# zjwzcx/A-2D-LiDAR-based-SLAM-System-for-Wheeled-Mobile-Robots

Hardware: AMD Instinct MI355X
Metric: scans/sec (360-beam ICP + 0.05 m grid update) (higher is better)
Workload: dtype f64; 1 GPU; configs[1]: 1000-scan replay (every 5th message of a 10 Hz stream, seed 1), 360 beams, ICP(max_iter=30, tol=0.001) + 400x400@0.05m grid, f64 point buffers; 32 independent replays of the 1000-scan trajectory per step (one slam_replay_dev call: ranges [32, 1000, 360], a map per trajectory); point_buffers=f64, pipeline=0, lanes=2, grid_mode=1, grid_group=16, parallelism=1 trajectory per GPU (32 independent replays of it per step)

## Files before the change

### a-2d-lidar-based-slam-system-for-wheeled-mobile-robots_amd/csrc/grid_kernels.hip

```cpp
#include <hip/hip_runtime.h>

#include <algorithm>
#include <mutex>
#include <utility>
#include <vector>
#include <climits>
#include <type_traits>

#include "slam_internal.h"
#include "slam_stamps.h"
#include "grid_walk.h"

namespace slam {

__device__ __forceinline__ unsigned cast_ray(uint32_t *__restrict__ pass, uint32_t *__restrict__ hit, int xw, int yw,
                                             int pcx, int pcy, int pox, int poy, bool &first_pending)
{
    Ray r;
    first_pending = false;
    if (!ray_setup(pcx, pcy, pox, poy, r)) return 0u;
    unsigned nvis = 0;
    double error = 0.0;
    int y = r.y0;
    for (int k = 0; k <= r.dx; ++k) {
        int x = r.x0 + k;
        int lx = r.steep ? y : x, ly = r.steep ? x : y;
        bool last = r.flag ? (k == 0) : (k == r.dx);
        bool first = r.flag ? (k == r.dx) : (k == 0);
        if ((unsigned)lx < (unsigned)xw && (unsigned)ly < (unsigned)yw) {
            ++nvis;
            if (first && lx == pcx && ly == pcy) {
                first_pending = true;
            } else {
                size_t c = (size_t)lx * yw + ly;
                atomicAdd(last ? &hit[c] : &pass[c], 1u);
            }
        }
        if (walk_step(error, r.derr)) y += r.ystep;
    }
    return nvis;
}

__device__ __forceinline__ unsigned wave_sum_u32(unsigned v)
{
#pragma unroll
    for (int off = 32; off > 0; off >>= 1) v += __shfl_xor(v, off, kWave);
    return v;
}

__device__ __forceinline__ int wave_or_i32(int v)
{
#pragma unroll
    for (int off = 32; off > 0; off >>= 1) v |= __shfl_xor(v, off, kWave);
    return v;
}

__device__ __forceinline__ void finish_wave(const GridDev &g, uint32_t *pass, int pcx, int pcy, bool first_pending,
                                            unsigned nvis, int bad)
{
    unsigned long long m = __ballot(first_pending);
    unsigned tot = wave_sum_u32(nvis);
    const int anybad = wave_or_i32(bad);
    if ((threadIdx.x & 63) == 0) {
        if (m) atomicAdd(&pass[(size_t)pcx * g.yw + pcy], (unsigned)__popcll(m));
        if (tot) atomicAdd(visit_slot(g.visits), (unsigned long long)tot);
        if (anybad) atomicOr(g.status, anybad);
    }
}

__device__ __forceinline__ void owner_fence() { asm volatile("s_waitcnt vmcnt(0)" ::: "memory"); }
constexpr int kWinCells = 36864;
constexpr int kWinMaxGroup = 64;
constexpr int kSortBins = 128;
constexpr int kMaxSortRays = 8192;
constexpr int kRaysPerLane = 4;

struct ScanConst {
    double px, py, c, s;
    int pcx, pcy, cbad, pad;
};

struct ReplaySource {
    const float *ranges;
    const double *cos_t, *sin_t, *poses;
    int n_scan, n;
    long traj_stride;
    int grid_per_traj;
    const double *centres;
    const double *heading_cs = nullptr;
    __device__ int scans_per_traj() const { return n_scan - 1; }
    __device__ int own_grid(int l) const { return grid_per_traj ? l : 0; }
    bool maps_are_private() const { return grid_per_traj != 0; }
    ReplaySource trajectories_from(int l0) const
    {
        ReplaySource r = *this;
        const size_t k = (size_t)l0 * (n_scan - 1);
        r.ranges += (size_t)l0 * traj_stride; r.poses += 3 * k;
        if (centres) r.centres += 2 * k;
        if (heading_cs) r.heading_cs += 2 * k;
        return r;
    }
    ReplaySource scans_from(int k0, int cnt) const
    {
        ReplaySource r = *this;
        r.ranges += (size_t)k0 * n; r.poses += 3 * (size_t)k0;
        if (centres) r.centres += 2 * (size_t)k0;
        if (heading_cs) r.heading_cs += 2 * (size_t)k0;
        r.n_scan = cnt + 1;
        return r;
    }
    __device__ void scan_const(int l, int k, const GridDev &g, ScanConst &sc) const
    {
        const double *pose = poses + 3 * ((size_t)l * (n_scan - 1) + k);
        sc.px = pose[0]; sc.py = pose[1];
        if (heading_cs) {
            const double *cs = heading_cs + 2 * ((size_t)l * (n_scan - 1) + k);
            sc.c = cs[0]; sc.s = cs[1];
        } else {
            sc.c = cos(pose[2]); sc.s = sin(pose[2]);
        }
        sc.cbad = 0;
        double ox = sc.px, oy = sc.py;
        if (centres) {
            const double *ctr = centres + 2 * ((size_t)l * (n_scan - 1) + k);
            ox = ctr[0]; oy = ctr[1];
        }
        sc.pcx = to_cell(ox, g.scale, g.off_x, sc.cbad);
        sc.pcy = to_cell(oy, g.scale, g.off_y, sc.cbad);
    }
    struct Beam { float r; double ct, st; };
    __device__ Beam fetch(int l, int k, int i) const
    {
        return Beam{ranges[(size_t)l * traj_stride + (size_t)(k + 1) * n + i], cos_t[i], sin_t[i]};
    }
    __device__ bool ray(const Beam &b, const ScanConst &sc, const GridDev &g, int &pox, int &poy, int &bad) const
    {
        double rr = (double)b.r;
        if (rr == INFINITY) rr = 30.0;
        double lx = b.ct * rr, ly = b.st * rr;
        double x = sc.c * lx + (-sc.s) * ly + sc.px * 1.0;
        double y = sc.s * lx + sc.c * ly + sc.py * 1.0;
        if (fabs(x) == INFINITY) return false;
        pox = to_cell(x, g.scale, g.off_x, bad);
        poy = to_cell(y, g.scale, g.off_y, bad);
        bad |= sc.cbad;
        return !bad;
    }
    __device__ bool ray(int l, int k, int i, const ScanConst &sc, const GridDev &g, int &pox, int &poy, int &bad) const
    {
        return ray(fetch(l, k, i), sc, g, pox, poy, bad);
    }
};

struct ExplicitSource {
    const double *ox, *oy, *cx, *cy;
    int B, n;
    __device__ int scans_per_traj() const { return B; }
    __device__ int own_grid(int) const { return 0; }
    bool maps_are_private() const { return false; }
// ... 54 lines not shown
        if (i < n && i <= stop && src.ray(l, k, i, sc, g, pox, poy, bad))
            nvis = cast_ray(pass, hit, g.xw, g.yw, sc.pcx, sc.pcy, pox, poy, first_pending);
        finish_wave(g, pass, sc.pcx, sc.pcy, first_pending, nvis, bad);
    }
}

typedef __attribute__((address_space(3))) unsigned lds_u32_t;
__device__ __forceinline__ unsigned lds_addr(const void *p)
{
    return (unsigned)(uintptr_t)(__attribute__((address_space(3))) const void *)p;
}
__device__ __forceinline__ void lds_add_u32(unsigned addr, unsigned v)
{
    (void)__hip_atomic_fetch_add((lds_u32_t *)(uintptr_t)addr, v, __ATOMIC_RELAXED, __HIP_MEMORY_SCOPE_WORKGROUP);
}

__device__ __forceinline__ int wave_min_i32(int v)
{
#pragma unroll
    for (int off = 32; off > 0; off >>= 1) v = min(v, __shfl_xor(v, off, kWave));
    return v;
}
__device__ __forceinline__ int wave_max_i32(int v)
{
#pragma unroll
    for (int off = 32; off > 0; off >>= 1) v = max(v, __shfl_xor(v, off, kWave));
    return v;
}

__device__ __forceinline__ void lds_walk(unsigned a, int da_k, int da_y, int rem, double derr, double &error, bool lead_in)
{
    auto advance = [&]() {
        const bool stepy = walk_step(error, derr);
        a += (unsigned)(da_k + (stepy ? da_y : 0));
    };
    auto step = [&]() {
        lds_add_u32(a & ~3u, 1u << ((a << 3) & 31u));
        advance();
    };
    if (lead_in) advance();
    for (;;) {
        const bool full = rem >= 4;
        if (!__any(full)) break;
        if (full) { step(); step(); step(); step(); rem -= 4; }
    }
#pragma unroll
    for (int u = 0; u < 3; ++u)
        if (rem > u) step();
}

__device__ __forceinline__ bool next_rays(int *next_ray, int nrays, const unsigned short *order, int &r)
{
    const int lane = threadIdx.x & 63;
    int base = 0;
    if (lane == 0) base = atomicAdd(next_ray, kWave);
    base = __builtin_amdgcn_readfirstlane(base);
    if (base >= nrays) return false;
    r = base + lane >= nrays ? -1 : order ? (int)order[base + lane] : base + lane;
    return true;
}

template <bool COVERS, class Src>
__device__ __forceinline__ unsigned cast_rays(const GridDev &g, const Src &src, const ScanConst *sc, int l, int s0, int n,
                                              int nrays, int *next_ray, const unsigned short *order, unsigned *win, int wx0,
                                              int wy0, int W, int H, int Hp2, uint32_t *__restrict__ pass,
                                              uint32_t *__restrict__ hit, const int *first_bad)
{
    unsigned nvis = 0;
    for (int r; next_rays(next_ray, nrays, order, r);) {
        if (r < 0) continue;
        int s = r / n, i = r - s * n, pox, poy, b2 = 0;
        Ray ry;
        if (i >= first_bad[s]) continue;
        if (!src.ray(l, s0 + s, i, sc[s], g, pox, poy, b2)) continue;
        if (!ray_setup(sc[s].pcx, sc[s].pcy, pox, poy, ry)) continue;
        CellWalk w(ry);
        int hx = -1, hy = -1;
        const int Hs = 2 * Hp2;
        const bool safe = (unsigned)(sc[s].pcx - wx0) < (unsigned)W && (unsigned)(sc[s].pcy - wy0) < (unsigned)H &&
                    (unsigned)(pox - wx0) < (unsigned)W && (unsigned)(poy - wy0) < (unsigned)H;
        if (!__any(!safe)) {
            const unsigned a2 = lds_addr(win) + 2u * (unsigned)((w.lx - wx0) * Hs + (w.ly - wy0));
            nvis += (unsigned)ry.dx + 1u;
            lds_walk(a2, 2 * w.stride_k(Hs), 2 * w.stride_y(Hs), ry.dx, w.derr, w.error, ry.flag);
            atomicAdd(&hit[(size_t)pox * g.yw + poy], 1u);
            continue;
        }
        for (int k = 0; k <= ry.dx; ++k, w.next()) {
            const int lx = w.lx, ly = w.ly;
            bool last = k == w.klast;
            unsigned wx = (unsigned)(lx - wx0), wy = (unsigned)(ly - wy0);
            bool inwin = wx < (unsigned)W && wy < (unsigned)H;
            bool inmap = COVERS ? inwin : ((unsigned)lx < (unsigned)g.xw && (unsigned)ly < (unsigned)g.yw);
            nvis += inmap ? 1u : 0u;
            hx = last ? lx : hx; hy = last ? ly : hy;
            if (inwin && !last) atomicAdd(&win[wx * Hp2 + (wy >> 1)], 1u << ((wy & 1u) * 16u));
            if (!COVERS) { if (inmap && !inwin && !last) atomicAdd(&pass[(size_t)lx * g.yw + ly], 1u); }
        }
        if ((unsigned)hx < (unsigned)g.xw && (unsigned)hy < (unsigned)g.yw) atomicAdd(&hit[(size_t)hx * g.yw + hy], 1u);
    }
    return nvis;
}

template <class Src>
__device__ __forceinline__ unsigned cast_rays_strip(const GridDev &g, const Src &src, const ScanConst &sc, int l, int s0,
                                                    int nrays, int *next_ray, const unsigned short *order, unsigned *win,
                                                    int wx0, int wy0, int W, int H, int Hp2, uint32_t *__restrict__ hit,
                                                    int first_bad)
{
    unsigned nvis = 0;
    for (int i; next_rays(next_ray, nrays, order, i);) {
        if (i < 0) continue;
        int pox, poy, b2 = 0;
        Ray ry;
        if (i >= first_bad) continue;
        if (!src.ray(l, s0, i, sc, g, pox, poy, b2)) continue;
        if (max(sc.pcx, pox) < wx0 || min(sc.pcx, pox) >= wx0 + W) continue;
        if (!ray_setup(sc.pcx, sc.pcy, pox, poy, ry)) continue;
        CellWalk w(ry);
        for (int k = 0; k <= ry.dx; ++k, w.next()) {
            const unsigned wx = (unsigned)(w.lx - wx0), wy = (unsigned)(w.ly - wy0);
            if (wx < (unsigned)W && wy < (unsigned)H) {
                ++nvis;
                unsigned *cell = &win[wx * Hp2 + (wy >> 1)];
                const unsigned sh = (wy & 1u) * 16u;
                if (k != w.klast) atomicAdd(cell, 1u << sh);
                else { atomicOr(cell, 0x8000u << sh); atomicAdd(&hit[(size_t)w.lx * g.yw + w.ly], 1u); }
            }
        }
    }
    return nvis;
}

struct WinCtl {
    int bbox[4];
    int qbox[4][4];
    int next_ray;
    int strips, strip_w;
    int phases, parity;
    alignas(8) unsigned long long visits;
    int first_bad[kWinMaxGroup];
    int phw[4][8];
    int phq[4];
    int seg[5];
};
constexpr int kWinBoxInts = 160;
static_assert(sizeof(WinCtl) <= kWinBoxInts * 4 && alignof(WinCtl) <= 16, "the control block outgrew its LDS region");
__host__ __device__ inline size_t win_sc_bytes(int group) { return ((size_t)group * sizeof(ScanConst) + 15) & ~(size_t)15; }
__host__ __device__ inline int win_sort_cap(long rays) { return rays <= kMaxSortRays ? (int)((rays + 7) & ~7L) : 0; }
__host__ __device__ inline size_t win_lds_bytes(int group, int sort_cap, int win_cells)
{
    return win_sc_bytes(group) + kWinBoxInts * 4 + 4 * kSortBins * 4 + (size_t)sort_cap * 2 + (size_t)win_cells * 2 + kLdsGuard;
}
inline int win_cells_for(int group, int sort_cap)
{
    const long half = 80 * 1024 - 512;
    long other = (long)win_lds_bytes(group, sort_cap, 0);
    long cells = ((half - other) / 2) & ~15L;
    return cells > kWinCells ? (int)cells : kWinCells;
}

struct WinLds {
    ScanConst *sc; WinCtl *ctl; int *hist; unsigned short *order; unsigned *win; char *guard;
    __device__ __forceinline__ WinLds(char *smem, int group_size, int sort_cap, int win_cells)
        : sc(reinterpret_cast<ScanConst *>(smem)),
          ctl(reinterpret_cast<WinCtl *>(smem + win_sc_bytes(group_size))),
          hist(reinterpret_cast<int *>(ctl) + kWinBoxInts),
          order(reinterpret_cast<unsigned short *>(hist + 4 * kSortBins)),
          win(reinterpret_cast<unsigned *>(order + sort_cap)),
          guard(reinterpret_cast<char *>(win) + (size_t)win_cells * 2) {}
};

template <class Src, class Park>
__device__ __forceinline__ void win_pass1(const GridDev &g, const Src &src, const ScanConst *sc, int l, int s0, int cnt, int n,
                                          bool sorted, int *bbox, int *first_bad, Park &&park)
{
    const int tid = threadIdx.x;
    int bx0 = INT_MAX, by0 = INT_MAX, bx1 = INT_MIN, by1 = INT_MIN;
    for (int r = tid; r < cnt * n; r += blockDim.x) {
        int s = r / n, i = r - s * n, pox, poy, len = 0, b2 = 0, quad = 0;
        const bool valid = src.ray(l, s0 + s, i, sc[s], g, pox, poy, b2);
        if (valid) {
            quad = (pox >= sc[s].pcx ? 1 : 0) | (poy >= sc[s].pcy ? 2 : 0);
            const int rx0 = min(pox, sc[s].pcx), rx1 = max(pox, sc[s].pcx), ry0 = min(poy, sc[s].pcy), ry1 = max(poy, sc[s].pcy);
            bx0 = min(bx0, rx0); bx1 = max(bx1, rx1);
            by0 = min(by0, ry0); by1 = max(by1, ry1);
            len = max(abs(pox - sc[s].pcx), abs(poy - sc[s].pcy));
        }
        if (b2) atomicMin(&first_bad[s], i);
        if (sorted) park(r, i, valid && len > 0, quad, kSortBins - 1 - min(len >> 2, kSortBins - 1));
    }
    bx0 = wave_min_i32(bx0); by0 = wave_min_i32(by0); bx1 = wave_max_i32(bx1); by1 = wave_max_i32(by1);
    if ((tid & 63) == 0 && bx0 <= bx1) {
        atomicMin(&bbox[0], bx0); atomicMin(&bbox[1], by0); atomicMax(&bbox[2], bx1); atomicMax(&bbox[3], by1);
    }
    __syncthreads();
    if (tid < cnt && first_bad[tid] != INT_MAX) {
        int pox, poy, b2 = 0;
        (void)src.ray(l, s0 + tid, first_bad[tid], sc[tid], g, pox, poy, b2);
        atomicOr(g.status, b2);
    }
}

template <int kBinsPerLane>
__device__ __forceinline__ void counting_sort(int *hist, const unsigned short *bins, unsigned short *order, int nrays, int *seg)
{
    constexpr int kLanesPerSeg = kSortBins / kBinsPerLane;
    const int lane = threadIdx.x & 63;
    if (threadIdx.x < kWave) {
        int h[kBinsPerLane], tot = 0;
#pragma unroll
        for (int u = 0; u < kBinsPerLane; ++u) { h[u] = hist[kBinsPerLane * lane + u]; tot += h[u]; }
        int inc = tot;
#pragma unroll
        for (int off = 1; off < kWave; off <<= 1) { int v = __shfl_up(inc, off, kWave); if (lane >= off) inc += v; }
        int run = inc - tot;
        if (seg && lane % kLanesPerSeg == 0) seg[lane / kLanesPerSeg] = run;
        if (seg && lane == kWave - 1) seg[kWave / kLanesPerSeg] = inc;
#pragma unroll
        for (int u = 0; u < kBinsPerLane; ++u) { hist[kBinsPerLane * lane + u] = run; run += h[u]; }
    }
    __syncthreads();
    for (int r = threadIdx.x; r < nrays; r += blockDim.x)
        if (bins[r] != 0xffffu) order[atomicAdd(&hist[bins[r]], 1)] = (unsigned short)r;
    __syncthreads();
}

__device__ __forceinline__ bool clamp_box(const GridDev &g, int *o, int ymask)
{
    o[0] = max(o[0], 0); o[1] = max(o[1], 0); o[2] = min(o[2], g.xw - 1); o[3] = min(o[3], g.yw - 1);
    o[1] &= ~ymask;
    return o[0] <= o[2] && o[1] <= o[3];
}
__device__ __forceinline__ bool box_fits(const int *o, int win_cells)
{
    return (long)(o[2] - o[0] + 1) * ((o[3] - o[1] + 2) & ~1) <= win_cells;
}

__device__ __forceinline__ void fit_window(const GridDev &g, bool any, const int *o, int ymask, const ScanConst &first, int win_cells, int *w)
{
    int x0 = any ? o[0] : 0, y0 = any ? o[1] : 0, W = any ? o[2] - o[0] + 1 : 0, H = any ? o[3] - o[1] + 1 : 0, cov = 1;
    if (any && !box_fits(o, win_cells)) {
        const int Hd = min(H, 192), Wd = min(W, win_cells / ((Hd + 1) & ~1));
        x0 = min(max(first.pcx - Wd / 2, o[0]), o[2] - Wd + 1);
        y0 = min(max(first.pcy - Hd / 2, o[1]), o[3] - Hd + 1) & ~ymask;
        W = Wd; H = Hd; cov = 0;
    }
    if ((long)W * ((H + 1) >> 1) > win_cells / 2) { atomicOr(g.status, kStatusGuard); W = 0; H = 0; cov = 0; }
    w[0] = x0; w[1] = y0; w[2] = W; w[3] = H; w[4] = cov;
}

__device__ __forceinline__ void flush_window(const unsigned *win, uint32_t *pass, int yw, int wx0, int wy0, int W, int Hp2, bool pair64)
{
    const int lane = threadIdx.x & 63, wave = threadIdx.x >> 6, nwaves = blockDim.x >> 6;
    const int rot = W > 0 ? (int)((blockIdx.x * 37u + blockIdx.y * 11u) % (unsigned)W) : 0;
    for (int rr = wave; rr < W; rr += nwaves) {
        const int row = rr + rot < W ? rr + rot : rr + rot - W;
        size_t gbase = (size_t)(wx0 + row) * yw + wy0;
        if (pair64 && (wy0 & 1) == 0) {
            for (int d = lane; d < Hp2; d += kWave) {
                unsigned v = win[row * Hp2 + d];
                if (v) atomicAdd(reinterpret_cast<unsigned long long *>(&pass[gbase + 2 * d]),
                                 (unsigned long long)(v & 0xffffu) | ((unsigned long long)(v >> 16) << 32));
            }
            continue;
        }
        for (int d = lane; d < Hp2; d += kWave) {
            unsigned v = win[row * Hp2 + d];
            unsigned p0 = v & 0xffffu, p1 = v >> 16;
            if (p0) atomicAdd(&pass[gbase + 2 * d], p0);
            if (p1) atomicAdd(&pass[gbase + 2 * d + 1], p1);
        }
    }
}

__device__ __forceinline__ void sweep_strip(const unsigned *win, uint32_t *pass, int8_t *pm, int yw, int sx0, int wy0, int SW, int H,
                                            int qrow, unsigned qinv, uint32_t pthr)
{
    const int tid = threadIdx.x, lane = tid & 63, Hp2 = H >> 1, total = SW * qrow;
    constexpr int kBatch = 4;
    for (int q0 = tid; q0 < total; q0 += kBatch * blockDim.x) {
        uint4 p[kBatch];
        uint32_t om[kBatch], d0[kBatch], d1[kBatch];
        size_t at[kBatch];
        bool live[kBatch];
#pragma unroll
        for (int u = 0; u < kBatch; ++u) {
            const int q = q0 + u * (int)blockDim.x;
            d0[u] = d1[u] = 0u;
            if (q < total) {
                const int r = (int)__umulhi((unsigned)q, qinv), c = q - r * qrow;
                const uint2 d = *reinterpret_cast<const uint2 *>(win + (r * Hp2 + 2 * c));
                d0[u] = d.x; d1[u] = d.y;
                at[u] = (size_t)(sx0 + r) * yw + (wy0 + 4 * c);
            }
            const unsigned long long m = __ballot((d0[u] | d1[u]) != 0u);
            live[u] = ((m >> (lane & 60)) & 0xFull) != 0ull;
            if (live[u]) {
                p[u] = *reinterpret_cast<const uint4 *>(pass + at[u]);
                om[u] = *reinterpret_cast<const uint32_t *>(pm + at[u]);
            }
        }
#pragma unroll
        for (int u = 0; u < kBatch; ++u) {
            if (!live[u]) continue;
            const uint32_t d0v = d0[u], d1v = d1[u];
            p[u].x += d0v & 0x7fffu; p[u].y += (d0v >> 16) & 0x7fffu; p[u].z += d1v & 0x7fffu; p[u].w += (d1v >> 16) & 0x7fffu;
            *reinterpret_cast<uint4 *>(pass + at[u]) = p[u];
            if (!(d0v | d1v)) continue;
            const uint32_t o = om[u];
            const uint32_t tb = ((d0v & 0xffffu) ? 1u : 0u) | ((d0v >> 16) ? 0x100u : 0u) | ((d1v & 0xffffu) ? 0x10000u : 0u) | ((d1v >> 16) ? 0x1000000u : 0u);
            const uint32_t fb = ((d0v >> 15) & 1u) | (((d0v >> 31) & 1u) << 8) | (((d1v >> 15) & 1u) << 16) | ((d1v >> 31) << 24);
            const uint32_t was = (o >> 6) & 0x01010101u, fresh = (o >> 4) & 0x01010101u;
            const uint32_t pmax = max(max(p[u].x, p[u].y), max(p[u].z, p[u].w));
            if (((tb & ~was) & (fresh | fb)) != 0u || pmax >= pthr) {
                uint32_t occ = was | fb;
                occ |= (p[u].x >= pthr ? 1u : 0u) | (p[u].y >= pthr ? 0x100u : 0u) | (p[u].z >= pthr ? 0x10000u : 0u) | (p[u].w >= pthr ? 0x1000000u : 0u);
                const uint32_t tm = tb * 255u;
                const uint32_t out = (o & ~tm) | ((occ * 100u) & tm);
                if (out != o) *reinterpret_cast<uint32_t *>(pm + at[u]) = out;
            }
        }
    }
}

__device__ __forceinline__ void finish_workgroup(const GridDev &g, unsigned long long *wg_visits, unsigned nvis, int tid)
{
    const unsigned tot = wave_sum_u32(nvis);
    if ((tid & 63) == 0 && tot) atomicAdd(wg_visits, (unsigned long long)tot);
    __syncthreads();
    if (tid == 0 && *wg_visits) atomicAdd(visit_slot(g.visits), *wg_visits);
}

template <class Src>
__global__ void __launch_bounds__(1024) k_grid_update_win(GridDev g, Src src, int group_size, const int32_t *__restrict__ got,
                                                          int sort_cap, int win_cells, int split)
{
    extern __shared__ __attribute__((aligned(16))) char smem[];
    const WinLds lds(smem, group_size, sort_cap, win_cells);
    ScanConst *sc = lds.sc; WinCtl *ctl = lds.ctl; int *hist = lds.hist; unsigned *win = lds.win;
    lds_guard_fill(lds.guard);
    STAMP_DECL;

    const int tid = threadIdx.x;
    const int l = blockIdx.y;
    const int my_half = split ? (int)(blockIdx.x & 1u) : -1;
    const int s0 = (int)(split ? blockIdx.x >> 1 : blockIdx.x) * group_size;
    const int cnt = min(group_size, src.scans_per_traj() - s0);
    const int gi = got ? got[l] : src.own_grid(l);
    uint32_t *pass = g.pass + (size_t)gi * g.xw * g.yw, *hit = g.hit + (size_t)gi * g.xw * g.yw;
    const int n = src.n, nrays = cnt * n;

    const bool pair64 = (g.yw & 1) == 0 && (((size_t)gi * g.xw * g.yw) & 1) == 0;
    const int ymask = pair64 ? 1 : 0;
    if (tid < cnt) { src.scan_const(l, s0 + tid, g, sc[tid]); ctl->first_bad[tid] = INT_MAX; }
    if (tid == 0) {
        ctl->bbox[0] = ctl->bbox[1] = INT_MAX; ctl->bbox[2] = ctl->bbox[3] = INT_MIN; ctl->next_ray = 0; ctl->visits = 0ull;
        for (int q = 0; q < 4; ++q) { ctl->qbox[q][0] = ctl->qbox[q][1] = INT_MAX; ctl->qbox[q][2] = ctl->qbox[q][3] = INT_MIN; }
        ctl->phases = 1; ctl->parity = 0;
    }
    const bool sorted = nrays <= sort_cap;
    unsigned short *bins = reinterpret_cast<unsigned short *>(win);
    for (int k = tid; k < 4 * kSortBins; k += blockDim.x) hist[k] = 0;
    __syncthreads();
    STAMP(0);

    win_pass1(g, src, sc, l, s0, cnt, n, sorted, ctl->bbox, ctl->first_bad, [&](int r, int i, bool casts, int quad, int lbin) {
        bins[r] = casts ? (unsigned short)(lbin | (quad << 7) | ((i & 1) << 9)) : (unsigned short)0xffffu;
    });
    if (tid == 0) {
        const int *bb = ctl->bbox;
        if (bb[0] <= bb[2]) {
            int ox0 = INT_MAX, oy0 = INT_MAX, ox1 = INT_MIN, oy1 = INT_MIN;
            for (int k = 0; k < cnt; ++k) { ox0 = min(ox0, sc[k].pcx); ox1 = max(ox1, sc[k].pcx); oy0 = min(oy0, sc[k].pcy); oy1 = max(oy1, sc[k].pcy); }
            for (int q = 0; q < 4; ++q) {
                ctl->qbox[q][0] = (q & 1) ? max(ox0, bb[0]) : bb[0]; ctl->qbox[q][2] = (q & 1) ? bb[2] : min(ox1, bb[2]);
                ctl->qbox[q][1] = (q & 2) ? max(oy0, bb[1]) : bb[1]; ctl->qbox[q][3] = (q & 2) ? bb[3] : min(oy1, bb[3]);
            }
        }
        auto box_of = [&](unsigned mask, int *o) -> bool {
            o[0] = o[1] = INT_MAX; o[2] = o[3] = INT_MIN;
            for (int q = 0; q < 4; ++q) {
                const int *b = ctl->qbox[q];
                if ((mask >> q & 1u) && b[0] <= b[2]) { o[0] = min(o[0], b[0]); o[1] = min(o[1], b[1]); o[2] = max(o[2], b[2]); o[3] = max(o[3], b[3]); }
            }
            return clamp_box(g, o, ymask);
        };
        auto fits = [&](unsigned mask) -> bool { int o[4]; return !box_of(mask, o) || box_fits(o, win_cells); };
        unsigned part[4] = {0u, 0u, 0u, 0u};
        int nph = 1, parity = 0;
        if (split) {
            const unsigned mine = my_half ? 0xAu : 0x5u;
            if (fits(0xFu)) { part[0] = 0xFu; parity = 1; }
            else if (fits(mine)) part[0] = mine;
            else { part[0] = mine & 0x3u; part[1] = mine & 0xCu; nph = 2; }
        } else {
            if (!sorted || fits(0xFu)) part[0] = 0xFu;
            else if (fits(0x5u) && fits(0xAu)) { part[0] = 0x5u; part[1] = 0xAu; nph = 2; }
            else { part[0] = 1u; part[1] = 2u; part[2] = 4u; part[3] = 8u; nph = 4; }
        }
        for (int q = 0; q < 4; ++q) ctl->phq[q] = -1;
        for (int ph = 0; ph < nph; ++ph) {
            for (int q = 0; q < 4; ++q)
                if (part[ph] >> q & 1u) ctl->phq[q] = ph;
            int o[4];
            const bool any = box_of(part[ph], o);
            fit_window(g, any, o, ymask, sc[0], win_cells, ctl->phw[ph]);
        }
        ctl->phases = nph; ctl->parity = parity;
        if (!sorted) { ctl->seg[0] = 0; ctl->seg[1] = nrays; }
    }
    __syncthreads();
    STAMP(1);
    const int phases = ctl->phases;
    if (sorted) {
        const bool parity = ctl->parity != 0;
        for (int r = tid; r < nrays; r += blockDim.x) {
            const unsigned b = bins[r];
            if (b == 0xffffu) continue;
            const int ph = ctl->phq[(b >> 7) & 3u];
            const bool mine = ph >= 0 && (!parity || (int)((b >> 9) & 1u) == my_half);
            const unsigned fin = (unsigned)ph * kSortBins + (b & 127u);
            bins[r] = mine ? (unsigned short)fin : (unsigned short)0xffffu;
            if (mine) atomicAdd(&hist[fin], 1);
        }
        __syncthreads();
        counting_sort<8>(hist, bins, lds.order, nrays, ctl->seg);
    }
    unsigned nvis = 0;
    int W = ctl->phw[0][2], H = ctl->phw[0][3];
    bool covers = ctl->phw[0][4] != 0;
    for (int ph = 0; ph < phases; ++ph) {
        const int seg0 = ctl->seg[ph], seg1 = ctl->seg[ph + 1];
        if (seg0 == seg1) continue;
        const int *o = ctl->phw[ph];
        const int wx0 = o[0], wy0 = o[1];
        W = o[2]; H = o[3]; covers = o[4] != 0;
        const int Hp2 = (H + 1) >> 1;
        __syncthreads();
        if (tid == 0) ctl->next_ray = 0;
        for (int w = tid; w < W * Hp2; w += blockDim.x) win[w] = 0u;
        __syncthreads();
        STAMP(2);
        const unsigned short *ord = sorted ? lds.order + seg0 : nullptr;
        if (covers) nvis += cast_rays<true>(g, src, sc, l, s0, n, seg1 - seg0, &ctl->next_ray, ord, win, wx0, wy0, W, H, Hp2, pass, hit, ctl->first_bad);
        else        nvis += cast_rays<false>(g, src, sc, l, s0, n, seg1 - seg0, &ctl->next_ray, ord, win, wx0, wy0, W, H, Hp2, pass, hit, ctl->first_bad);
        __syncthreads();
        STAMP(3);
        flush_window(win, pass, g.yw, wx0, wy0, W, Hp2, pair64);
    }
    finish_workgroup(g, &ctl->visits, nvis, tid);
    STAMP(4);
    STAMP_VAL((ctl->parity << 8) | (covers ? 1 : 0) | (phases << 4) | ((unsigned)(W * ((H + 1) & ~1)) << 12));
    STAMP_END(5);
    lds_guard_check(lds.guard, g.status);
}

template <class Src>
__global__ void __launch_bounds__(1024) k_grid_update_own(GridDev g, Src src, int group_size, int sort_cap, int win_cells)
{
    extern __shared__ __attribute__((aligned(16))) char smem[];
    const WinLds lds(smem, group_size, sort_cap, win_cells);
    ScanConst *sc = lds.sc; WinCtl *ctl = lds.ctl; int *hist = lds.hist; unsigned *win = lds.win;
    lds_guard_fill(lds.guard);
    STAMP_DECL;

    const int tid = threadIdx.x, lane = tid & 63, wave = tid >> 6, nwaves = blockDim.x >> 6;
    const int l = blockIdx.y;
    const int s0 = (int)blockIdx.x * group_size;
    const int cnt = min(group_size, src.scans_per_traj() - s0);
    const int gi = src.own_grid(l);
    uint32_t *pass = g.pass + (size_t)gi * g.xw * g.yw, *hit = g.hit + (size_t)gi * g.xw * g.yw;
    int8_t *pm = g.pmap_live + (size_t)gi * g.xw * g.yw;
    const int n = src.n, nrays = cnt * n;

    const bool fused = (g.yw & 3) == 0 && (((size_t)gi * g.xw * g.yw) & 3) == 0;
    const bool pair64 = (g.yw & 1) == 0 && (((size_t)gi * g.xw * g.yw) & 1) == 0;
    const int ymask = fused ? 3 : pair64 ? 1 : 0;
    if (tid < cnt) { src.scan_const(l, s0 + tid, g, sc[tid]); ctl->first_bad[tid] = INT_MAX; }
    if (tid == 0) {
        ctl->bbox[0] = ctl->bbox[1] = INT_MAX; ctl->bbox[2] = ctl->bbox[3] = INT_MIN; ctl->next_ray = 0; ctl->visits = 0ull;
        ctl->strips = 0; ctl->strip_w = 0;
    }
    const bool sorted = nrays <= sort_cap;
    unsigned short *bins = reinterpret_cast<unsigned short *>(win);
    for (int k = tid; k < kSortBins; k += blockDim.x) hist[k] = 0;
    __syncthreads();
    STAMP(0);

    win_pass1(g, src, sc, l, s0, cnt, n, sorted, ctl->bbox, ctl->first_bad, [&](int r, int, bool, int, int lbin) {
        bins[r] = (unsigned short)lbin;
        atomicAdd(&hist[lbin], 1);
    });
    if (tid == 0) {
        int o[4] = {ctl->bbox[0], ctl->bbox[1], ctl->bbox[2], ctl->bbox[3]};
        int *w = ctl->phw[0];
        const bool any = clamp_box(g, o, 0);
        if (any && fused && cnt == 1 && nrays < 32768 && g.hit_levels == 1 && (g.yw & 15) == 0) {
            const int ya = o[1] & ~15, Ha = ((o[3] | 15) + 1) - ya, Wb = o[2] - o[0] + 1;
            int S = (int)(((long)Wb * Ha + win_cells - 1) / win_cells), Ws = (Wb + S - 1) / S;
            while ((long)Ws * Ha > win_cells && S < Wb) { ++S; Ws = (Wb + S - 1) / S; }
            if ((long)Ws * Ha <= win_cells) { w[0] = o[0]; w[1] = ya; w[2] = Wb; w[3] = Ha; w[4] = 1; ctl->strips = S; ctl->strip_w = Ws; }
        }
        if (!ctl->strips) {
            o[1] &= ~ymask;
            fit_window(g, any, o, ymask, sc[0], win_cells, w);
        }
    }
    __syncthreads();
    STAMP(1);
    if (sorted) counting_sort<kSortBins / kWave>(hist, bins, lds.order, nrays, nullptr);
    const unsigned short *ord = sorted ? lds.order : nullptr;
    const int wx0 = ctl->phw[0][0], wy0 = ctl->phw[0][1], W = ctl->phw[0][2], H = ctl->phw[0][3];
    const bool covers = ctl->phw[0][4] != 0;
    const int Hp2 = (H + 1) >> 1;
    const int strips = ctl->strips, strip_w = ctl->strip_w;
    unsigned nvis = 0;
    if (strips) {
        const uint32_t pthr = g.pass_thresh[0];
        const int qrow = H >> 2;
        const unsigned qinv = (unsigned)((0x100000000ull + (unsigned)qrow - 1) / (unsigned)qrow);
        for (int strip = 0; strip < strips; ++strip) {
            const int sx0 = wx0 + strip * strip_w, SW = min(strip_w, wx0 + W - sx0);
            if (strip) __syncthreads();
            for (int w = tid; w < SW * Hp2; w += blockDim.x) win[w] = 0u;
            if (tid == 0) ctl->next_ray = 0;
            __syncthreads();
            STAMP(2);
            nvis += cast_rays_strip(g, src, sc[0], l, s0, nrays, &ctl->next_ray, ord, win, sx0, wy0, SW, H, Hp2, hit, ctl->first_bad[0]);
            __syncthreads();
            STAMP(3);
            sweep_strip(win, pass, pm, g.yw, sx0, wy0, SW, H, qrow, qinv, pthr);
            STAMP_SYNC();
            STAMP(4);
        }
        STAMP_COUNT(7, strips);
    } else {
        for (int w = tid; w < W * Hp2; w += blockDim.x) win[w] = 0u;
        __syncthreads();
        STAMP(2);
        if (covers) nvis += cast_rays<true>(g, src, sc, l, s0, n, nrays, &ctl->next_ray, ord, win, wx0, wy0, W, H, Hp2, pass, hit, ctl->first_bad);
        else        nvis += cast_rays<false>(g, src, sc, l, s0, n, nrays, &ctl->next_ray, ord, win, wx0, wy0, W, H, Hp2, pass, hit, ctl->first_bad);
        __syncthreads();
        STAMP(3);
        if (!fused) flush_window(win, pass, g.yw, wx0, wy0, W, Hp2, pair64);
        owner_fence();
        __syncthreads();
        const int x0 = max(ctl->bbox[0], 0), y0 = max(ctl->bbox[1], 0), x1 = min(ctl->bbox[2], g.xw - 1), y1 = min(ctl->bbox[3], g.yw - 1);
        const OccRule rule = OccRule::of(g);
        if (x0 <= x1 && y0 <= y1 && fused) {
            const int ya = y0 & ~3, qrow = ((y1 | 3) + 1 - ya) >> 2, rows = x1 - x0 + 1;
            const int total = rows * qrow;
// ... 410 lines not shown
    const int x0 = min(box[0], c0.pcx), y0 = min(box[1], c0.pcy), x1 = max(box[2], c0.pcx), y1 = max(box[3], c0.pcy);
    const int y4 = y0 & ~15, Hs = ((y1 | 15) + 1) - y4, W = x1 - x0 + 1;
    if ((long)W * Hs > (long)win_bytes) { give_up(); return; }
    {
        const int excl = inc - (h0 + h1);
        int base = __shfl(excl, bin >> 1, kWave);
        const int first = __shfl(h0, bin >> 1, kWave);
        if (bin & 1) base += first;
        if (valid) slots[base + idx] = pk;
    }
    __syncthreads();
    STAMP(2);

    const bool have = tid < nv;
    const unsigned e = have ? slots[tid] : 0u;
    const int ex = (int)(e & 0xffffu), ey = (int)(e >> 16);
    Ray rr = Ray::none();
    if (have) (void)ray_setup(c0.pcx, c0.pcy, ex, ey, rr);
    const unsigned wbase = lds_addr(win);
    if (have) {
        const unsigned b = (unsigned)((ex - x0) * Hs + (ey - y4));
        lds_or_u32(wbase + (b & ~3u), 0x80u << ((b & 3u) * 8u));
    }
    {
        CellWalk w(rr);
        const unsigned a = wbase + (unsigned)((w.lx - x0) * Hs + (w.ly - y4));
        lds_walk(a, w.stride_k(Hs), w.stride_y(Hs), have ? rr.dx - 1 : 0, w.derr, w.error, have);
    }
    __syncthreads();
    STAMP(3);

    const int wv = __builtin_amdgcn_readfirstlane(tid >> 6);
    constexpr int NW = THREADS / kWave;
    const int qrow = Hs >> 2, nseg = (qrow + kWave - 1) >> 6;

    {
        unsigned acc = 0u;
        for (int seg = 0; seg < nseg; ++seg) {
            const int c = seg * kWave + lane;
            if (c < qrow)
                for (int r = wv; r < W; r += NW) acc = __builtin_amdgcn_sad_u8(win[r * qrow + c] & 0x7f7f7f7fu, 0u, acc);
        }
        acc = wave_sum_u32(acc);
        if (lane == 0 && acc) atomicAdd(&box[6], (int)acc);
    }
    __syncthreads();
    if (box[6] != box[5]) { give_up(); return; }

    uint32_t *pass = g.pass + (size_t)gi * g.xw * g.yw, *hit = g.hit + (size_t)gi * g.xw * g.yw;
    int8_t *pm = g.pmap_live + (size_t)gi * g.xw * g.yw;
    if (tid == 0) atomicAdd(visit_slot(g.visits), (unsigned long long)(box[5] + 2 * nv));

    const uint32_t pthr = g.pass_thresh[0];
    const int org_r = c0.pcx - x0, org_q = (c0.pcy - y4) >> 2;
    const unsigned org_b = (unsigned)(c0.pcy - y4) & 3u;
    const __amdgpu_buffer_rsrc_t rs_pass = __builtin_amdgcn_make_buffer_rsrc(pass, 0, g.xw * g.yw * 4, kBufferRsrcWord3);
    const __amdgpu_buffer_rsrc_t rs_pm = __builtin_amdgcn_make_buffer_rsrc(pm, 0, g.xw * g.yw, kBufferRsrcWord3);
    constexpr unsigned kSkip = 0x80000000u;
    for (int seg = 0; seg < nseg; ++seg) {
        const int c = seg * kWave + lane;
        const bool incol = c < qrow;
        const bool org_lane = c == org_q;
        for (int r0 = wv; r0 < W; r0 += NW * BATCH) {
            u32x4_t p[BATCH];
            uint32_t om[BATCH], dd[BATCH], vo[BATCH], vp[BATCH], ev[BATCH];
            auto rowoff_of = [&](int u) -> uint32_t {
                const int rc = min(r0 + u * NW, W - 1);
                return (uint32_t)((x0 + rc) * g.yw + y4 + seg * 4 * kWave);
            };
#pragma unroll
            for (int u = 0; u < BATCH; ++u) {
                const int r = r0 + u * NW;
                const int rc = min(r, W - 1);
                dd[u] = (incol && r < W) ? win[rc * qrow + c] : 0u;
                const unsigned long long m = __ballot(dd[u] != 0u || (r == org_r && org_lane));
                const bool live = ((m >> (lane & 60)) & 0xFull) != 0ull && incol;
                vo[u] = live ? (unsigned)lane << 4 : kSkip;
                p[u] = __builtin_amdgcn_raw_buffer_load_b128(rs_pass, vo[u], rowoff_of(u) << 2, kOwn8Aux);
            }
#pragma unroll
            for (int u = 0; u < BATCH; ++u) {
                vp[u] = (vo[u] != kSkip && (dd[u] & 0x80808080u) != 0u) ? (unsigned)lane << 2 : kSkip;
                om[u] = __builtin_amdgcn_raw_buffer_load_b32(rs_pm, vp[u], rowoff_of(u), kOwn8Aux);
            }
            bool late_any = false;
#pragma unroll
            for (int u = 0; u < BATCH; ++u) {
                const int r = r0 + u * NW;
                const uint32_t d = dd[u], dm = d & 0x7f7f7f7fu;
                u32x4_t q = p[u];
                const uint32_t z7 = (q.x == 0u ? 0x80u : 0u) | (q.y == 0u ? 0x8000u : 0u) | (q.z == 0u ? 0x800000u : 0u) | (q.w == 0u ? 0x80000000u : 0u);
                q.x += dm & 0xffu; q.y += (dm >> 8) & 0xffu; q.z += (dm >> 16) & 0xffu; q.w += dm >> 24;
                uint32_t t7 = ((dm + 0x7f7f7f7fu) | d) & 0x80808080u;
                if (r == org_r) {
                    if (org_lane) {
                        q.x += org_b == 0u ? (uint32_t)nv : 0u; q.y += org_b == 1u ? (uint32_t)nv : 0u;
                        q.z += org_b == 2u ? (uint32_t)nv : 0u; q.w += org_b == 3u ? (uint32_t)nv : 0u;
                        t7 |= 0x80u << (8u * org_b);
                    }
                }
                __builtin_amdgcn_raw_buffer_store_b128(q, rs_pass, vo[u], rowoff_of(u) << 2, kOwn8Aux);
                const uint32_t ge5 = (q.x >= pthr ? 0x20u : 0u) | (q.y >= pthr ? 0x2000u : 0u) | (q.z >= pthr ? 0x200000u : 0u) | (q.w >= pthr ? 0x20000000u : 0u);
                ev[u] = t7 | ((d >> 1) & 0x40404040u) | ge5;
                if (vp[u] == kSkip && vo[u] != kSkip && ((t7 & z7) != 0u || (ge5 & (t7 >> 2)) != 0u)) {
                    vp[u] = ((unsigned)lane << 2) | 1u;
                    late_any = true;
                }
            }
#pragma unroll
            for (int u = 0; u < BATCH; ++u) {
                if (vp[u] == kSkip || (vp[u] & 1u)) continue;
                const uint32_t out = own8_pmap_bytes(om[u], ev[u]);
                if (out != om[u]) __builtin_amdgcn_raw_buffer_store_b32(out, rs_pm, vp[u], rowoff_of(u), kOwn8Aux);
            }
            if (__any(late_any)) {
#pragma unroll
                for (int u = 0; u < BATCH; ++u)
                    om[u] = __builtin_amdgcn_raw_buffer_load_b32(rs_pm, (vp[u] != kSkip && (vp[u] & 1u)) ? vp[u] & ~3u : kSkip, rowoff_of(u), kOwn8Aux);
#pragma unroll
                for (int u = 0; u < BATCH; ++u) {
                    if (vp[u] == kSkip || !(vp[u] & 1u)) continue;
                    const uint32_t out = own8_pmap_bytes(om[u], ev[u]);
                    if (out != om[u]) __builtin_amdgcn_raw_buffer_store_b32(out, rs_pm, vp[u] & ~3u, rowoff_of(u), kOwn8Aux);
                }
            }
        }
    }
    if (have) atomicAdd(&hit[(size_t)ex * g.yw + ey], 1u);
    STAMP_SYNC();
    STAMP(4);
    STAMP_END(5);
    lds_guard_check(guard, g.status);
}

struct ChipShape { int cus; long lds_per_cu; };
static ChipShape chip_shape()
{
    static std::mutex mu;
    static std::vector<std::pair<int, ChipShape>> seen;
    int dev = 0;
    ChipShape c{256, 160 * 1024};
    if (hipGetDevice(&dev) != hipSuccess) return c;
    std::lock_guard<std::mutex> lock(mu);
    for (const auto &e : seen)
        if (e.first == dev) return e.second;
    int v = 0;
    if (hipDeviceGetAttribute(&v, hipDeviceAttributeMultiprocessorCount, dev) == hipSuccess && v > 0) c.cus = v;
    if (hipDeviceGetAttribute(&v, hipDeviceAttributeMaxSharedMemoryPerMultiprocessor, dev) == hipSuccess && v > 0) c.lds_per_cu = v;
    (void)hipGetLastError();
    seen.push_back({dev, c});
    return c;
}

template <class Src>
static hipError_t launch_win(const GridDev &g, const Src &src, int L, int scans, int n, int group, const int32_t *got,
                             hipStream_t s, int split_pref = -1)
{
    const size_t lds_max = win_lds_bytes(kWinMaxGroup, kMaxSortRays, kWinCells);
    for (const void *f : {reinterpret_cast<const void *>(&k_grid_update_win<Src>), reinterpret_cast<const void *>(&k_grid_update_own<Src>)}) {
        hipError_t e = allow_dynamic_lds(f, (int)lds_max);
        if (e != hipSuccess) return e;
    }
    int groups = (scans + group - 1) / group;
    long rays = (long)group * n;
    long want = (rays + kRaysPerLane - 1) / kRaysPerLane;
    int threads = want >= kMaxWaves * kWave ? kMaxWaves * kWave : (int)(((want + kWave - 1) / kWave) * kWave);
    if (threads < 128) threads = 128;
    const int exclusive = g.pmap_live && groups == 1 && !got && (L == 1 || src.maps_are_private());
    if (g.pmap_live && !exclusive && g.live_dirty) *g.live_dirty = true;
    constexpr int kWinMinThreads = 512;
    if (threads < kWinMinThreads) threads = kWinMinThreads;
    const int sort_cap = win_sort_cap((long)group * n);
    const int win_cells = win_cells_for(group, sort_cap);
    if (exclusive && group == 1 && scans == 1 && g.hit_levels == 1 && (g.yw & 15) == 0 && (((size_t)g.xw * g.yw) & 3) == 0 &&
        g.yw <= win_cells && n <= kOwnerMaxRays * kOwnerThreads) {
        for (const void *f : {reinterpret_cast<const void *>(&k_grid_update_owner<Src, 1>), reinterpret_cast<const void *>(&k_grid_update_owner<Src, 2>),
                              reinterpret_cast<const void *>(&k_grid_update_owner_redo<Src, 1>)}) {
            hipError_t e = allow_dynamic_lds(f, (int)lds_max);
            if (e != hipSuccess) return e;
        }
        const size_t lds = win_lds_bytes(1, sort_cap, win_cells);
        if (g.redo && n <= kOwn8Threads && n <= kOwnerThreads && g.xw <= 65535 && g.yw <= 65535 && (long)g.xw * g.yw < (1L << 29)) {
            const int own8_lds = kOwn8LdsBytes + kLdsGuard, own8_win = (int)(kOwn8LdsBytes - own8_fixed_bytes(kOwn8Threads));
            SLAM_LAUNCH((k_grid_update_owner8<Src, kOwn8Threads, kOwn8Batch>), dim3(1, L), dim3(kOwn8Threads), own8_lds, s,
                        g, src, own8_win, g.redo);
            SLAM_LAUNCH((k_grid_update_owner_redo<Src, 1>), dim3(std::min(L, 256)), dim3(kOwnerThreads), lds, s, g, src, sort_cap, win_cells, g.redo);
            return hipGetLastError();
        }
        if (n <= kOwnerThreads) SLAM_LAUNCH((k_grid_update_owner<Src, 1>), dim3(1, L), dim3(kOwnerThreads), lds, s, g, src, sort_cap, win_cells);
        else                    SLAM_LAUNCH((k_grid_update_owner<Src, 2>), dim3(1, L), dim3(kOwnerThreads), lds, s, g, src, sort_cap, win_cells);
        return hipGetLastError();
    }
    const ChipShape chip = chip_shape();
    const int split = (!exclusive && sort_cap > 0 && (split_pref > 0 || (split_pref < 0 && (long)groups * L <= (3L * chip.cus) / 4))) ? 1 : 0;
    size_t lds = win_lds_bytes(group, sort_cap, win_cells);
    const long wgs = (long)(split ? 2 * groups : groups) * L;
    const size_t half_cu = (size_t)(chip.lds_per_cu / 2);
    if (split && wgs <= chip.cus && lds <= half_cu && half_cu + 512 <= (size_t)chip.lds_per_cu) lds = half_cu + 512;
    if (lds > lds_max) {
        const void *f = exclusive ? reinterpret_cast<const void *>(&k_grid_update_own<Src>) : reinterpret_cast<const void *>(&k_grid_update_win<Src>);
        hipError_t e = allow_dynamic_lds(f, (int)lds);
        if (e != hipSuccess) return e;
    }
    if (exclusive) SLAM_LAUNCH((k_grid_update_own<Src>), dim3(groups, L), dim3(threads), lds, s, g, src, group, sort_cap, win_cells);
    else SLAM_LAUNCH((k_grid_update_win<Src>), dim3(split ? 2 * groups : groups, L), dim3(threads), lds, s, g, src, group, got,
                     sort_cap, win_cells, split);
    return hipGetLastError();
}

static int pick_group(int group, long total_scans, int scans_per_traj, int n)
{
    int gmax = std::min(kWinMaxGroup, 65535 / std::max(n, 1));
    if (gmax < 1) return 0;
    if (group <= 0) {
        long want = (total_scans + 127) / 128;
        group = (int)std::min<long>(std::max<long>(want, 1), 12);
    }
    group = std::min(std::min(group, gmax), std::max(scans_per_traj, 1));
    return group;
}

constexpr int kTileSteps = 2048;
constexpr int kTileWords = kTileSteps / 32;
constexpr int kTileSide = 192;

struct RayRec {
    int x0, y0, dx, yend;
    uint32_t flags;
    int pad[3];
};

struct TileScratch {
    RayRec *recs;
    uint32_t *bits;
    unsigned short *prefix;
    int *gbox;
};

__global__ void __launch_bounds__(256) k_tile_init(int *gbox, int groups)
{
    int i = blockIdx.x * blockDim.x + threadIdx.x;
    if (i < groups) { gbox[4 * i] = gbox[4 * i + 1] = INT_MAX; gbox[4 * i + 2] = gbox[4 * i + 3] = INT_MIN; }
}

template <class Src>
__global__ void __launch_bounds__(256) k_ray_bits(GridDev g, Src src, TileScratch ts, int group_size)
{
    __shared__ ScanConst sc;
    __shared__ int box[4];
    const int s = blockIdx.x, l = blockIdx.y, n = src.n;
    const int scans = src.scans_per_traj();
    const int groups_per_traj = (scans + group_size - 1) / group_size;
    const int group = l * groups_per_traj + s / group_size;
    uint32_t *pass = g.pass, *hit = g.hit;
    __shared__ int first_bad;
    if (threadIdx.x == 0) {
        src.scan_const(l, s, g, sc);
        box[0] = box[1] = INT_MAX; box[2] = box[3] = INT_MIN;
        first_bad = INT_MAX;
    }
    __syncthreads();
    for (int i = threadIdx.x; i < n; i += blockDim.x) {
        int pox, poy, b2 = 0;
        (void)src.ray(l, s, i, sc, g, pox, poy, b2);
        if (b2) atomicMin(&first_bad, i);
    }
    __syncthreads();
    const int stop = first_bad;
    unsigned nvis = 0;
    int bad = 0;
    for (int i = threadIdx.x; i < n; i += blockDim.x) {
        const size_t rid = ((size_t)l * scans + s) * n + i;
        RayRec rec;
        rec.flags = 0; rec.x0 = rec.y0 = rec.dx = rec.yend = 0; rec.pad[0] = rec.pad[1] = rec.pad[2] = 0;
        int pox, poy, b2 = 0;
        Ray ry;
        const bool valid = i <= stop && src.ray(l, s, i, sc, g, pox, poy, b2) && ray_setup(sc.pcx, sc.pcy, pox, poy, ry);
        const bool plain = valid && ry.dx < kTileSteps && (unsigned)sc.pcx < (unsigned)g.xw && (unsigned)sc.pcy < (unsigned)g.yw &&
                           (unsigned)pox < (unsigned)g.xw && (unsigned)poy < (unsigned)g.yw;
        {
            uint32_t *bw = ts.bits + rid * kTileWords;
            unsigned short *pw = ts.prefix + rid * kTileWords;
            const int dx = plain ? ry.dx : -1;
            const double derr = plain ? ry.derr : 0.0;
            double error = 0.0;
            uint32_t count = 0, before_last = 0;
            for (int k0 = 0; __any(k0 <= dx); k0 += 32) {
                if (k0 <= dx) {
                    uint32_t word = 0;
                    const int nb = min(32, dx - k0 + 1);
#pragma unroll 8
                    for (int b = 0; b < 32; ++b) {
                        word |= walk_step(error, derr) ? (1u << b) : 0u;
                    }
                    if (nb < 32) word &= (1u << nb) - 1u;
                    pw[k0 >> 5] = (unsigned short)count;
                    bw[k0 >> 5] = word;
                    if (k0 + 32 > dx) before_last = count + __popc(word & ((1u << (dx - k0)) - 1u));
                    count += __popc(word);
                }
            }
            if (plain) {
                nvis += (unsigned)ry.dx + 1u;
                atomicAdd(&hit[(size_t)pox * g.yw + poy], 1u);
                rec.yend = ry.y0 + ry.ystep * (int)before_last;
                rec.x0 = ry.x0; rec.y0 = ry.y0; rec.dx = ry.dx;
                rec.flags = 8u | (ry.steep ? 1u : 0u) | (ry.flag ? 2u : 0u) | (ry.ystep > 0 ? 4u : 0u);
                int a0 = ry.x0, a1 = ry.x0 + ry.dx, b0 = min(ry.y0, rec.yend), b1 = max(ry.y0, rec.yend);
                int mx0 = ry.steep ? b0 : a0, mx1 = ry.steep ? b1 : a1, my0 = ry.steep ? a0 : b0, my1 = ry.steep ? a1 : b1;
                atomicMin(&box[0], mx0); atomicMin(&box[1], my0); atomicMax(&box[2], mx1); atomicMax(&box[3], my1);
            }
        }
        if (valid && !plain) {
            const bool record = ry.dx < kTileSteps;
            uint32_t *bw = ts.bits + rid * kTileWords;
            unsigned short *pw = ts.prefix + rid * kTileWords;
            const int klast = ry.flag ? 0 : ry.dx;
            double error = 0.0;
            int y = ry.y0, hx = -1, hy = -1;
            uint32_t word = 0, count = 0;
            for (int k = 0; k <= ry.dx; ++k) {
                if (record && (k & 31) == 0) pw[k >> 5] = (unsigned short)count;
                int x = ry.x0 + k;
                int lx = ry.steep ? y : x, ly = ry.steep ? x : y;
                bool inmap = (unsigned)lx < (unsigned)g.xw && (unsigned)ly < (unsigned)g.yw;
                nvis += inmap ? 1u : 0u;
                if (k == klast) { hx = lx; hy = ly; }
                else if (!record && inmap) atomicAdd(&pass[(size_t)lx * g.yw + ly], 1u);
                if (k == ry.dx) rec.yend = y;
                if (walk_step(error, ry.derr)) { y += ry.ystep; word |= 1u << (k & 31); ++count; }
                if (record && ((k & 31) == 31 || k == ry.dx)) { bw[k >> 5] = word; word = 0; }
            }
            if ((unsigned)hx < (unsigned)g.xw && (unsigned)hy < (unsigned)g.yw) atomicAdd(&hit[(size_t)hx * g.yw + hy], 1u);
            if (record) {
                rec.x0 = ry.x0; rec.y0 = ry.y0; rec.dx = ry.dx;
                rec.flags = 8u | (ry.steep ? 1u : 0u) | (ry.flag ? 2u : 0u) | (ry.ystep > 0 ? 4u : 0u);
                int a0 = ry.x0, a1 = ry.x0 + ry.dx, b0 = min(ry.y0, rec.yend), b1 = max(ry.y0, rec.yend);
                int mx0 = ry.steep ? b0 : a0, mx1 = ry.steep ? b1 : a1, my0 = ry.steep ? a0 : b0, my1 = ry.steep ? a1 : b1;
                atomicMin(&box[0], mx0); atomicMin(&box[1], my0); atomicMax(&box[2], mx1); atomicMax(&box[3], my1);
            }
        }
        bad |= b2;
        ts.recs[rid] = rec;
    }
    __syncthreads();
    if (threadIdx.x == 0 && box[0] <= box[2]) {
        atomicMin(&ts.gbox[4 * group], box[0]); atomicMin(&ts.gbox[4 * group + 1], box[1]);
        atomicMax(&ts.gbox[4 * group + 2], box[2]); atomicMax(&ts.gbox[4 * group + 3], box[3]);
    }
    unsigned tot = wave_sum_u32(nvis);
    int anybad = bad;
#pragma unroll
    for (int off = 32; off > 0; off >>= 1) anybad |= __shfl_xor(anybad, off, kWave);
    if ((threadIdx.x & 63) == 0) {
        if (tot) atomicAdd(visit_slot(g.visits), (unsigned long long)tot);
        if (anybad) atomicOr(g.status, anybad);
// ... 742 lines not shown
```

Measured before the change: 18.64 million scans/s.

## Shrink grid window LDS so two workgroups fit per CU, add 3-phase split

When there are more window workgroups than CUs, the window size is computed from half the real per-CU LDS so two workgroups can be resident per CU. It also sets a launch-bounds occupancy hint and adds three-phase quadrant partitions when only one half-window fits. An env-gated residency report is added. The smaller window can force more multi-phase passes over the rays, and the launch-bounds hint may limit registers.

```diff
diff --git a/a-2d-lidar-based-slam-system-for-wheeled-mobile-robots_amd/csrc/grid_kernels.hip b/a-2d-lidar-based-slam-system-for-wheeled-mobile-robots_amd/csrc/grid_kernels.hip
--- a/a-2d-lidar-based-slam-system-for-wheeled-mobile-robots_amd/csrc/grid_kernels.hip
+++ b/a-2d-lidar-based-slam-system-for-wheeled-mobile-robots_amd/csrc/grid_kernels.hip
@@ -5,6 +5,8 @@
 #include <utility>
 #include <vector>
 #include <climits>
+#include <cstdio>
+#include <cstdlib>
 #include <type_traits>
 
 #include "slam_internal.h"
@@ -365,13 +367,17 @@
 {
     return win_sc_bytes(group) + kWinBoxInts * 4 + 4 * kSortBins * 4 + (size_t)sort_cap * 2 + (size_t)win_cells * 2 + kLdsGuard;
 }
-inline int win_cells_for(int group, int sort_cap)
-{
-    const long half = 80 * 1024 - 512;
+constexpr int kWinHalfSlack = 512;
+constexpr int kWinTwoFloor = 29632;
+inline int win_cells_for(int group, int sort_cap, bool two_per_cu = false, long lds_per_cu = 160 * 1024)
+{
+    const long half = lds_per_cu / 2 - kWinHalfSlack;
     long other = (long)win_lds_bytes(group, sort_cap, 0);
     long cells = ((half - other) / 2) & ~15L;
-    return cells > kWinCells ? (int)cells : kWinCells;
-}
+    if (cells > kWinCells) return (int)cells;
+    return two_per_cu && cells >= kWinTwoFloor ? (int)cells : kWinCells;
+}
+static_assert(kWinTwoFloor >= kMaxSortRays && kWinTwoFloor % 16 == 0, "pass 1 parks a 16-bit key per sorted ray in the window");
 
 struct WinLds {
     ScanConst *sc; WinCtl *ctl; int *hist; unsigned short *order; unsigned *win; char *guard;
@@ -546,7 +552,7 @@
 }
 
 template <class Src>
-__global__ void __launch_bounds__(1024) k_grid_update_win(GridDev g, Src src, int group_size, const int32_t *__restrict__ got,
+__global__ void __launch_bounds__(1024, 8) k_grid_update_win(GridDev g, Src src, int group_size, const int32_t *__restrict__ got,
                                                           int sort_cap, int win_cells, int split)
 {
     extern __shared__ __attribute__((aligned(16))) char smem[];
@@ -609,8 +615,13 @@
             else { part[0] = mine & 0x3u; part[1] = mine & 0xCu; nph = 2; }
         } else {
             if (!sorted || fits(0xFu)) part[0] = 0xFu;
-            else if (fits(0x5u) && fits(0xAu)) { part[0] = 0x5u; part[1] = 0xAu; nph = 2; }
-            else { part[0] = 1u; part[1] = 2u; part[2] = 4u; part[3] = 8u; nph = 4; }
+            else {
+                const bool left = fits(0x5u), right = fits(0xAu);
+                if (left && right) { part[0] = 0x5u; part[1] = 0xAu; nph = 2; }
+                else if (left) { part[0] = 0x5u; part[1] = 2u; part[2] = 8u; nph = 3; }
+                else if (right) { part[0] = 1u; part[1] = 4u; part[2] = 0xAu; nph = 3; }
+                else { part[0] = 1u; part[1] = 2u; part[2] = 4u; part[3] = 8u; nph = 4; }
+            }
         }
         for (int q = 0; q < 4; ++q) ctl->phq[q] = -1;
         for (int ph = 0; ph < nph; ++ph) {
@@ -1327,6 +1338,17 @@
     return c;
 }
 
+static void report_win_residency(const void *kernel, int threads, size_t lds, int win_cells, long wgs)
+{
+    const char *on = getenv("SLAM_WIN_RESIDENCY");
+    if (!on || !*on || *on == '0') return;
+    int per_cu = -1;
+    const hipError_t e = hipOccupancyMaxActiveBlocksPerMultiprocessor(&per_cu, kernel, threads, lds);
+    if (e != hipSuccess) (void)hipGetLastError();
+    fprintf(stderr, "k_grid_update_win: %d threads, %zu bytes of LDS (window %d cells), %ld workgroups: %d resident per CU%s\n",
+            threads, lds, win_cells, wgs, per_cu, e == hipSuccess ? "" : " (the query failed)");
+}
+
 template <class Src>
 static hipError_t launch_win(const GridDev &g, const Src &src, int L, int scans, int n, int group, const int32_t *got,
                              hipStream_t s, int split_pref = -1)
@@ -1346,9 +1368,10 @@
     constexpr int kWinMinThreads = 512;
     if (threads < kWinMinThreads) threads = kWinMinThreads;
     const int sort_cap = win_sort_cap((long)group * n);
-    const int win_cells = win_cells_for(group, sort_cap);
+    const int own_cells = win_cells_for(group, sort_cap);
     if (exclusive && group == 1 && scans == 1 && g.hit_levels == 1 && (g.yw & 15) == 0 && (((size_t)g.xw * g.yw) & 3) == 0 &&
-        g.yw <= win_cells && n <= kOwnerMaxRays * kOwnerThreads) {
+        g.yw <= own_cells && n <= kOwnerMaxRays * kOwnerThreads) {
+        const int win_cells = own_cells;
         for (const void *f : {reinterpret_cast<const void *>(&k_grid_update_owner<Src, 1>), reinterpret_cast<const void *>(&k_grid_update_owner<Src, 2>),
                               reinterpret_cast<const void *>(&k_grid_update_owner_redo<Src, 1>)}) {
             hipError_t e = allow_dynamic_lds(f, (int)lds_max);
@@ -1368,8 +1391,9 @@
     }
     const ChipShape chip = chip_shape();
     const int split = (!exclusive && sort_cap > 0 && (split_pref > 0 || (split_pref < 0 && (long)groups * L <= (3L * chip.cus) / 4))) ? 1 : 0;
+    const long wgs = (long)(split ? 2 * groups : groups) * L;
+    const int win_cells = (!exclusive && sort_cap > 0 && wgs > chip.cus) ? win_cells_for(group, sort_cap, true, chip.lds_per_cu) : own_cells;
     size_t lds = win_lds_bytes(group, sort_cap, win_cells);
-    const long wgs = (long)(split ? 2 * groups : groups) * L;
     const size_t half_cu = (size_t)(chip.lds_per_cu / 2);
     if (split && wgs <= chip.cus && lds <= half_cu && half_cu + 512 <= (size_t)chip.lds_per_cu) lds = half_cu + 512;
     if (lds > lds_max) {
@@ -1377,6 +1401,7 @@
         hipError_t e = allow_dynamic_lds(f, (int)lds);
         if (e != hipSuccess) return e;
     }
+    if (!exclusive) report_win_residency(reinterpret_cast<const void *>(&k_grid_update_win<Src>), threads, lds, win_cells, wgs);
     if (exclusive) SLAM_LAUNCH((k_grid_update_own<Src>), dim3(groups, L), dim3(threads), lds, s, g, src, group, sort_cap, win_cells);
     else SLAM_LAUNCH((k_grid_update_win<Src>), dim3(split ? 2 * groups : groups, L), dim3(threads), lds, s, g, src, group, got,
                      sort_cap, win_cells, split);
```

New measurement: 18.89 million scans/s (median of 6 runs). 1.01x the previous value.
